# computational-cell-analytics/micro-sam

Hardware: AMD Instinct MI355X
Metric: 1024^2 tiles/s embed+AMG (vit_b bf16) (higher is better)
Workload: dtype bf16 image encoder (patch embedding + neck, 1.2 % of its flops, on hi+lo operand pairs of that type), fp16 mask decoder (16-bit MFMA operands, fp32 accumulation); 1 GPU; configs[1]: vit_b, 1024x1024 uint8 synthetic tiles, batched embedding precompute + AutomaticMaskGenerator (32x32 grid, multimask, default thresholds); encoder_batch=16, distinct_tiles_per_gpu=256, weights=seeded synthetic checkpoint (synthetic.py variant 'cells'), decode_lanes=3

## Files before the change

### micro_sam_amd/build.py

```python
import os
import subprocess
import sys

HERE = os.path.dirname(os.path.abspath(__file__))
CSRC = os.path.join(HERE, "csrc")
LIB_DIR = os.path.join(HERE, "lib")
LIB_PATH = os.path.join(LIB_DIR, "libmsam_hip.so")
SOURCES = ["gemm.hip", "norm.hip", "attention.hip", "decoder.hip", "postprocess.hip", "encoder.hip", "segment.hip", "wsgemm.hip", "declayer.hip", "decfold.hip", "decfold_tok.hip", "upfused.hip", "image.hip", "train.hip", "amgselect.hip", "watershed.hip", "strict.hip", "objfeat.hip", "matching.hip", "labelprops.hip", "propagate.hip", "embedpca.hip", "semloss.hip", "depthconv.hip"]
ARCH = "gfx950"


def _hipcc() -> str:
    for cand in (os.environ.get("HIPCC"), "/opt/rocm/bin/hipcc", "hipcc"):
        if cand and (os.path.isabs(cand) and os.path.exists(cand) or not os.path.isabs(cand)):
            return cand
    return "hipcc"


def needs_build() -> bool:
    if not os.path.exists(LIB_PATH):
        return True
    t = os.path.getmtime(LIB_PATH)
    deps = [os.path.join(CSRC, f) for f in os.listdir(CSRC)] + [os.path.join(HERE, "..", "include", "msam_hip.h")]
    return any(os.path.getmtime(d) > t for d in deps if os.path.exists(d))


def variant_path(variant: str = "") -> str:
    return LIB_PATH if not variant else os.path.join(LIB_DIR, f"libmsam_hip_{variant}.so")


def build(force: bool = False, verbose: bool = True, variant: str = "", experiments: bool = False) -> str:
    os.makedirs(LIB_DIR, exist_ok=True)
    marker = os.path.join(LIB_DIR, ".experiments")
    if experiments or os.path.exists(marker):
        force = True
        if experiments:
            open(marker, "w").close()
        else:
            os.remove(marker)
    if variant:
        return _build_variant(variant, force, verbose)
    if not force and not needs_build():
        return LIB_PATH
    objs = []
    for src in SOURCES:
        path = os.path.join(CSRC, src)
        if not os.path.exists(path):
            continue
        obj = os.path.join(LIB_DIR, src.replace(".hip", ".o"))
        if force or not os.path.exists(obj) or os.path.getmtime(obj) < max(
                os.path.getmtime(path), os.path.getmtime(os.path.join(CSRC, "common.h")),
                os.path.getmtime(os.path.join(HERE, "..", "include", "msam_hip.h"))):
            cmd = [_hipcc(), f"--offload-arch={ARCH}", "-O3", "-std=c++17", "-fPIC", "-c", path, "-o", obj]
            if experiments:
                cmd.insert(-4, "-DMSAM_EXPERIMENTS=1")
            if verbose:
                print(" ".join(cmd), flush=True)
            subprocess.check_call(cmd)
        objs.append(obj)
    cmd = [_hipcc(), f"--offload-arch={ARCH}", "-shared", "-fPIC", *objs, "-o", LIB_PATH]
    if verbose:
        print(" ".join(cmd), flush=True)
    subprocess.check_call(cmd)
    return LIB_PATH


def _build_variant(variant: str, force: bool, verbose: bool) -> str:
    if variant != "decbf16":
        raise ValueError(f"unknown build variant {variant!r}")
    out = variant_path(variant)
    deps = [os.path.join(CSRC, f) for f in os.listdir(CSRC)]
    if not force and os.path.exists(out) and all(os.path.getmtime(d) <= os.path.getmtime(out) for d in deps):
        return out
    objs = []
    for src in SOURCES:
        obj = os.path.join(LIB_DIR, src.replace(".hip", f".{variant}.o"))
        cmd = [_hipcc(), f"--offload-arch={ARCH}", "-O3", "-std=c++17", "-fPIC", "-DMSAM_DEC_F16=0", "-c", os.path.join(CSRC, src),
               "-o", obj]
        if verbose:
            print(" ".join(cmd), flush=True)
        subprocess.check_call(cmd)
        objs.append(obj)
    subprocess.check_call([_hipcc(), f"--offload-arch={ARCH}", "-shared", "-fPIC", *objs, "-o", out])
    return out


if __name__ == "__main__":
    print(build(force="--force" in sys.argv, variant="decbf16" if "--dec-bf16" in sys.argv else "", experiments="--experiments" in sys.argv))
```

### micro_sam_amd/csrc/decfold.hip

```cpp
#include "common.h"
#include "../../include/msam_hip.h"
#include <string>

void msam_set_error(const char* msg);
int msam_check_launch(const char* what);
void msam_profile_mark2(void* stream, int begin, double flops, double bytes, int family);

namespace {

constexpr int T = 4096, C = 256, CI = 128, TK = 32, NTHR = 256;
constexpr int SUBT = 1024 + 32;
constexpr int KEYS_BYTES = 16 * SUBT, TAB_BYTES = TK * CI * 2, BUF_BYTES = KEYS_BYTES + TAB_BYTES;
constexpr float NEG_BIG = -1.0e30f;
#ifndef FOLD_ATTN_DMA_DEFAULT
#define FOLD_ATTN_DMA_DEFAULT 0
#endif

typedef short s16x4_t __attribute__((ext_vector_type(4)));

MSAM_DEVINL uint2 lds_tr16(const unsigned char* p) {
    s16x4_t v = __builtin_amdgcn_ds_read_tr16_b64_v4i16((s16x4_t __attribute__((address_space(3)))*)p);
    return __builtin_bit_cast(uint2, v);
}

// ... 523 lines not shown
#undef FI_TAB
#undef I2T_STAMP
}

__global__ __launch_bounds__(256) void fold_v_kernel(const u16* __restrict__ vtok, const u16* __restrict__ wo, int Nt,
                                                     u16* __restrict__ vfoldT) {
    __shared__ float v[8][CI];
    const int p = blockIdx.x, c = threadIdx.x;
    for (int i = c; i < 8 * CI; i += 256) {
        const int t = i >> 7, d = i & (CI - 1);
        v[t][d] = t < Nt ? d2f(vtok[((long)p * Nt + t) * CI + d]) : 0.f;
    }
    __syncthreads();
    u16* dst = vfoldT + ((long)p * C + c) * 64;
    for (int h = 0; h < 8; ++h) {
        const uint4 w0 = *(const uint4*)(wo + (long)c * CI + h * 16), w1 = *(const uint4*)(wo + (long)c * CI + h * 16 + 8);
        const uint32_t ww[8] = {w0.x, w0.y, w0.z, w0.w, w1.x, w1.y, w1.z, w1.w};
        float wf[16];
#pragma unroll
        for (int x = 0; x < 8; ++x) { wf[2 * x] = d2f((u16)(ww[x] & 0xffff)); wf[2 * x + 1] = d2f((u16)(ww[x] >> 16)); }
        uint32_t pk[4];
#pragma unroll
        for (int t2 = 0; t2 < 4; ++t2) {
            float a0 = 0.f, a1 = 0.f;
#pragma unroll
            for (int d = 0; d < 16; ++d) { a0 = fmaf(wf[d], v[2 * t2][h * 16 + d], a0); a1 = fmaf(wf[d], v[2 * t2 + 1][h * 16 + d], a1); }
            pk[t2] = pack2d(a0, a1);
        }
        *(uint4*)(dst + h * 8) = make_uint4(pk[0], pk[1], pk[2], pk[3]);
    }
}

int key_splits(int P) {
    int ks = 1;
    while (P * ks < 512 && ks < 16) ks *= 2;
    return ks;
}

}

extern "C" int64_t msam_t2i_fold_workspace_bytes(int32_t P) {
    const long ks = key_splits(P);
    return (long)P * 64 * C * 2 + (long)P * ks * 64 * C * 4 + (long)P * ks * 64 * 2 * 4;
}

extern "C" int msam_t2i_fold_attention(const void* keys, int32_t kv_shared, const void* qtok, int32_t P, int32_t Nt,
                                       const void* wk, const void* tabk, const void* wv, const float* bv, void* out,
                                       void* workspace, int64_t workspace_bytes, void* stream) {
    if (!keys || !qtok || !wk || !tabk || !wv || !bv || !out || !workspace || P <= 0) {
        msam_set_error("msam_t2i_fold_attention: null argument");
        return 1;
    }
    if (Nt < 1 || Nt > 8) { msam_set_error("msam_t2i_fold_attention: 1 <= Nt <= 8 tokens per prompt"); return 1; }
    if (workspace_bytes < msam_t2i_fold_workspace_bytes(P)) { msam_set_error("msam_t2i_fold_attention: workspace too small"); return 1; }
    hipStream_t s = (hipStream_t)stream;
    const int KS = key_splits(P);
    char* wp = (char*)workspace;
    u16* qprime = (u16*)wp; wp += (long)P * 64 * C * 2;
    float* opart = (float*)wp; wp += (long)P * KS * 64 * C * 4;
    float* stats = (float*)wp;
    hipLaunchKernelGGL(fold_q_kernel, dim3(P * 8), dim3(256), 0, s, (const u16*)qtok, (const u16*)wk, Nt, qprime);
    if (int e = msam_check_launch("fold_q")) return e;
    FoldArgs a{};
    a.keys = (const u16*)keys; a.kv_shared = kv_shared & 1; a.blocked = (kv_shared >> 1) & 1; a.qprime = qprime; a.qtok = (const u16*)qtok; a.Nt = Nt;
    a.tabk = (const u16*)tabk; a.nitems = P * KS; a.KS = KS; a.opart = opart; a.stats = stats;
    a.wv = (const u16*)wv; a.bv = bv; a.out = (u16*)out;
    int dev = 0, cus = 256;
    (void)hipGetDevice(&dev);
    (void)hipDeviceGetAttribute(&cus, hipDeviceAttributeMultiprocessorCount, dev);
    const int grid = a.nitems < 2 * cus ? a.nitems : 2 * cus;
    const double flops = (double)P * T * (2.0 * 64 * C * 2 + 2.0 * 64 * 32);
    const double bytes = (double)((kv_shared & 1) ? 1 : P) * T * C * 2 + (KS > 1 ? (double)P * KS * 64 * C * 4 : 0.0);
    msam_profile_mark2(stream, 1, flops, bytes, 3);
    if (g_fold_attn_dma && !a.blocked) {
        const int grid3 = a.nitems < 3 * cus ? a.nitems : 3 * cus;
        hipLaunchKernelGGL(fold_attn_kernel<true>, dim3(grid3), dim3(NTHR), 0, s, a);
    } else {
        hipLaunchKernelGGL(fold_attn_kernel<false>, dim3(grid), dim3(NTHR), 0, s, a);
    }
    msam_profile_mark2(stream, 0, flops, bytes, 3);
    if (int e = msam_check_launch("fold_attn")) return e;
    if (KS == 1) return 0;
    hipLaunchKernelGGL(fold_finish_kernel, dim3(P * 8), dim3(128), 0, s, opart, stats, KS, Nt, (const u16*)wv, bv, (u16*)out);
    return msam_check_launch("fold_finish");
}

int64_t msam_i2t_tok_workspace_bytes(int32_t P);
int msam_i2t_tok_layer(const void* xin, int32_t x_shared, const void* ktok, const void* vtok, int32_t P, int32_t Nt,
                       const void* wq, const void* tabq, const void* wo, const float* bo, const float* ln_w,
                       const float* ln_b, float ln_eps, void* out, void* workspace, int KS, void* stream);
extern int g_tune_i2t_variant;

extern "C" int64_t msam_i2t_fold_workspace_bytes(int32_t P) {
    const int64_t a = (int64_t)P * 64 * C * 2 * 2, b = msam_i2t_tok_workspace_bytes(P);
    return a > b ? a : b;
}

extern "C" int msam_i2t_fold_layer(const void* xin, int32_t x_shared, const void* ktok, const void* vtok, int32_t P,
                                   int32_t Nt, const void* wq, const void* tabq, const void* wo, const float* bo,
                                   const float* ln_w, const float* ln_b, float ln_eps, void* out, void* workspace,
                                   int64_t workspace_bytes, void* stream) {
    if (!xin || !ktok || !vtok || !wq || !tabq || !wo || !bo || !ln_w || !ln_b || !out || !workspace || P <= 0) {
        msam_set_error("msam_i2t_fold_layer: null argument");
        return 1;
    }
    if (Nt < 1 || Nt > 8) { msam_set_error("msam_i2t_fold_layer: 1 <= Nt <= 8 tokens per prompt"); return 1; }
    if (workspace_bytes < msam_i2t_fold_workspace_bytes(P)) { msam_set_error("msam_i2t_fold_layer: workspace too small"); return 1; }
    if (g_tune_i2t_variant == 1)
        return msam_i2t_tok_layer(xin, x_shared, ktok, vtok, P, Nt, wq, tabq, wo, bo, ln_w, ln_b, ln_eps, out, workspace,
                                  key_splits(P), stream);
    hipStream_t s = (hipStream_t)stream;
    u16* kfold = (u16*)workspace;
    u16* vfoldT = kfold + (long)P * 64 * C;
    hipLaunchKernelGGL(fold_q_kernel, dim3(P * 8), dim3(256), 0, s, (const u16*)ktok, (const u16*)wq, Nt, kfold);
    if (int e = msam_check_launch("fold_k")) return e;
    hipLaunchKernelGGL(fold_v_kernel, dim3(P), dim3(256), 0, s, (const u16*)vtok, (const u16*)wo, Nt, vfoldT);
    if (int e = msam_check_launch("fold_v")) return e;
    I2tArgs a{};
    a.xin = (const u16*)xin; a.x_shared = x_shared; a.kfold = kfold; a.vfoldT = vfoldT; a.ktok = (const u16*)ktok; a.Nt = Nt;
    a.tabq = (const u16*)tabq; a.bo = bo; a.ln_w = ln_w; a.ln_b = ln_b; a.eps = ln_eps;
    a.KS = key_splits(P); a.nitems = P * a.KS; a.out = (u16*)out;
    int dev = 0, cus = 256;
    (void)hipGetDevice(&dev);
    (void)hipDeviceGetAttribute(&cus, hipDeviceAttributeMultiprocessorCount, dev);
    const int grid = a.nitems < 2 * cus ? a.nitems : 2 * cus;
    const double flops = (double)P * T * (2.0 * 64 * C * 2 + 2.0 * 64 * 32);
    const double bytes = (double)(x_shared ? 1 : P) * T * C * 2 + (double)P * T * C * 2;
    msam_profile_mark2(stream, 1, flops, bytes, 2);
    if (g_i2t_timing) hipLaunchKernelGGL(fold_i2t_kernel<true>, dim3(grid), dim3(NTHR), 0, s, a);
    else hipLaunchKernelGGL(fold_i2t_kernel<false>, dim3(grid), dim3(NTHR), 0, s, a);
    msam_profile_mark2(stream, 0, flops, bytes, 2);
    return msam_check_launch("fold_i2t");
}

extern "C" int msam_debug_i2t_timing(int32_t enable, uint64_t* host_out) {
    g_i2t_timing = enable;
    if (host_out) {
        if (hipDeviceSynchronize() != hipSuccess ||
            hipMemcpyFromSymbol(host_out, HIP_SYMBOL(g_i2t_stamps), sizeof(unsigned long long) * 64 * 12) != hipSuccess) {
            msam_set_error("msam_debug_i2t_timing: copy failed");
            return 2;
        }
    }
    return 0;
}

extern "C" int msam_fold_attn_set_dma(int32_t on) { g_fold_attn_dma = on; return 0; }

extern int g_tune_i2t_wg_per_cu, g_tune_chain_variant, g_tune_chain_tmask, g_tune_up_gelu16, g_tune_up_ln_two_pass, g_tune_up_centred;
void msam_gemm_set_dbg(int v);
void msam_gemm_set_gw(int delay, int cls);
void msam_gemm_set_g3(int delay);
void msam_gemm_set_g3_epi(int v);
extern int g_tune_tok_fuse;
extern int g_tune_mlp_split_fused;
extern int g_tune_sgemm_bufs, g_tune_srel_mfma, g_tune_sgemm_small_below, g_tune_si2t_dbg, g_tune_si2t_late_us, g_tune_sattn_allh;
int g_tune_dec_chain = 1, g_tune_dec_chain_min_p = 128;
extern "C" int msam_tune_set(const char* key, int32_t value) {
    const std::string k = key ? key : "";
    if (k == "i2t_variant") g_tune_i2t_variant = value;
    else if (k == "i2t_wg_per_cu") g_tune_i2t_wg_per_cu = value;
    else if (k == "dec_chain") g_tune_dec_chain = value;
    else if (k == "chain_variant") g_tune_chain_variant = value;
    else if (k == "chain_tmask") g_tune_chain_tmask = value;
    else if (k == "up_gelu16") g_tune_up_gelu16 = value;
    else if (k == "up_ln_two_pass") g_tune_up_ln_two_pass = value;
    else if (k == "up_centred") g_tune_up_centred = value;
    else if (k == "gemm_dbg") msam_gemm_set_dbg(value);
    else if (k == "gw_delay") msam_gemm_set_gw(value, -1);
    else if (k == "gw_class") msam_gemm_set_gw(-2, value);
    else if (k == "g3_delay") msam_gemm_set_g3(value);
    else if (k == "g3_epi") msam_gemm_set_g3_epi(value);
    else if (k == "tok_fuse") g_tune_tok_fuse = value;
    else if (k == "mlp_split_fused") g_tune_mlp_split_fused = value;
    else if (k == "dec_chain_min_p") g_tune_dec_chain_min_p = value;
    else if (k == "sgemm_bufs") g_tune_sgemm_bufs = value;
    else if (k == "srel_mfma") g_tune_srel_mfma = value;
    else if (k == "sattn_allh") g_tune_sattn_allh = value;
    else if (k == "sgemm_small_below") g_tune_sgemm_small_below = value;
    else if (k == "si2t_dbg") g_tune_si2t_dbg = value;
    else if (k == "si2t_late_us") g_tune_si2t_late_us = value;
    else { msam_set_error("msam_tune_set: unknown key"); return 1; }
    return 0;
}
```

### micro_sam_amd/csrc/gemm.hip

```cpp
#include <stdio.h>
#include <stdlib.h>
#include "common.h"
#include "../../include/msam_hip.h"

float* msam_det_workspace(size_t floats, int slot);
int msam_det_reduce(const float* parts, int nparts, long n, float* out, int accumulate, void* stream);

namespace {

constexpr int BM = 128, BN = 128, BK = 64;
constexpr int TILE_CHUNKS = BM * 8;

struct Epi {
    const float* bias; const float* table; int table_rows, table_cols; long table_ld;
    const void* resid; int resid_dtype, resid_rows; long ldr;
    int act;
    void* out; int out_dtype; long ldc;
    int out_mode; u16* q; u16* k; u16* v; int heads, head_dim, tokens;
    const float* row_scale; const float* col_scale;
    int splitk_len = 0;
    unsigned long long* trace = nullptr;
    int direct_epi = 0;
    int gw_delay = 0, gw_class = 0;
    int dbg = 0;
// ... 874 lines not shown
    } while (0)
#define LN_COMMIT(buf_)                                                                             \
    do {                                                                                            \
        uint4* la_ = ldsA + (buf_) * LM * 8; uint4* lb_ = ldsB + (buf_) * LN_ * 8;                  \
        la_[(0 * 32 + srow) * 8 + scp] = ra0; la_[(1 * 32 + srow) * 8 + scp] = ra1;                 \
        lb_[(0 * 32 + srow) * 8 + scp] = rw0; lb_[(1 * 32 + srow) * 8 + scp] = rw1;                 \
        lb_[(2 * 32 + srow) * 8 + scp] = rw2; lb_[(3 * 32 + srow) * 8 + scp] = rw3;                 \
        lb_[(4 * 32 + srow) * 8 + scp] = rw4; lb_[(5 * 32 + srow) * 8 + scp] = rw5;                 \
        lb_[(6 * 32 + srow) * 8 + scp] = rw6; lb_[(7 * 32 + srow) * 8 + scp] = rw7;                 \
    } while (0)
    LN_ISSUE(0);
    LN_COMMIT(0);
    __syncthreads();
    const int fr = lane & 15, fg = lane >> 4;
    for (int kt = 0; kt < nk; ++kt) {
        const int buf = kt & 1;
        if (kt + 1 < nk) LN_ISSUE(kt + 1);
        const uint4* la = ldsA + buf * LM * 8; const uint4* lb = ldsB + buf * LN_ * 8;
#pragma unroll
        for (int ks = 0; ks < 2; ++ks) {
            uint4 a[4], b[4];
#pragma unroll
            for (int i = 0; i < 4; ++i) {
                const int row = i * 16 + fr;
                a[i] = la[row * 8 + ((ks * 4 + fg) ^ swz(row))];
                const int col = wave * 64 + i * 16 + fr;
                b[i] = lb[col * 8 + ((ks * 4 + fg) ^ swz(col))];
            }
#pragma unroll
            for (int i = 0; i < 4; ++i)
#pragma unroll
                for (int j = 0; j < 4; ++j) acc[i][j] = F16 ? mfma16h(a[i], b[j], acc[i][j]) : mfma16(a[i], b[j], acc[i][j]);
        }
        if (kt + 1 < nk) LN_COMMIT(buf ^ 1);
        __syncthreads();
    }
#undef LN_ISSUE
#undef LN_COMMIT
    float* ldsC = (float*)dyn_lds;
#pragma unroll
    for (int i = 0; i < 4; ++i)
#pragma unroll
        for (int j = 0; j < 4; ++j)
#pragma unroll
            for (int r = 0; r < 4; ++r) ldsC[(i * 16 + fg * 4 + r) * LN_ + wave * 64 + j * 16 + fr] = acc[i][j][r];
    __syncthreads();

    const int col = lane * 4;
    float bias4[4] = {0.f, 0.f, 0.f, 0.f};
    if (e.bias) { float4 b = *(const float4*)(e.bias + col); bias4[0] = b.x; bias4[1] = b.y; bias4[2] = b.z; bias4[3] = b.w; }
    const bool use_table = e.table && col < e.table_cols;
    float lw[4] = {1.f, 1.f, 1.f, 1.f}, lb4[4] = {0.f, 0.f, 0.f, 0.f};
    if (ln.mode) {
        const int lc = ln.mode == 2 ? (col & 63) : col;
        float4 w4 = *(const float4*)(ln.ln_w + lc), b4 = *(const float4*)(ln.ln_b + lc);
        lw[0] = w4.x; lw[1] = w4.y; lw[2] = w4.z; lw[3] = w4.w; lb4[0] = b4.x; lb4[1] = b4.y; lb4[2] = b4.z; lb4[3] = b4.w;
    }
    for (int pass = 0; pass < 16; ++pass) {
        const int lr = pass * 4 + wave;
        const int row = m0 + lr;
        if (row >= M) break;
        float4 c = *(const float4*)(ldsC + lr * LN_ + col);
        float v[4] = {c.x + bias4[0], c.y + bias4[1], c.z + bias4[2], c.w + bias4[3]};
        if (use_table) {
            float4 t = *(const float4*)(e.table + (long)(row % e.table_rows) * e.table_ld + col);
            v[0] += t.x; v[1] += t.y; v[2] += t.z; v[3] += t.w;
        }
        if (e.resid_dtype) {
            const int rr = e.resid_rows ? (row % e.resid_rows) : row;
            if (e.resid_dtype == MSAM_F32) {
                float4 t = *(const float4*)((const float*)e.resid + (long)rr * e.ldr + col);
                v[0] += t.x; v[1] += t.y; v[2] += t.z; v[3] += t.w;
            } else {
                uint2 t = *(const uint2*)((const u16*)e.resid + (long)rr * e.ldr + col);
                v[0] += load16((u16)(t.x & 0xffff), e.resid_dtype); v[1] += load16((u16)(t.x >> 16), e.resid_dtype);
                v[2] += load16((u16)(t.y & 0xffff), e.resid_dtype); v[3] += load16((u16)(t.y >> 16), e.resid_dtype);
            }
        }
        if (ln.mode) {
            const float s = (v[0] + v[1]) + (v[2] + v[3]);
            const float inv_n = ln.mode == 1 ? (1.0f / 256.0f) : (1.0f / 64.0f);
            const float mean = (ln.mode == 1 ? wave_sum64(s) : wave_sum_xor16(s)) * inv_n;
            const float d0 = v[0] - mean, d1 = v[1] - mean, d2 = v[2] - mean, d3 = v[3] - mean;
            const float q = (d0 * d0 + d1 * d1) + (d2 * d2 + d3 * d3);
            const float var = (ln.mode == 1 ? wave_sum64(q) : wave_sum_xor16(q)) * inv_n;
            const float rstd = 1.0f / sqrtf(var + ln.eps);
            v[0] = d0 * rstd * lw[0] + lb4[0]; v[1] = d1 * rstd * lw[1] + lb4[1];
            v[2] = d2 * rstd * lw[2] + lb4[2]; v[3] = d3 * rstd * lw[3] + lb4[3];
            if (ln.mode == 2) { v[0] = gelu_erf(v[0]); v[1] = gelu_erf(v[1]); v[2] = gelu_erf(v[2]); v[3] = gelu_erf(v[3]); }
        }
        if (e.act == MSAM_ACT_GELU) { v[0] = gelu_erf(v[0]); v[1] = gelu_erf(v[1]); v[2] = gelu_erf(v[2]); v[3] = gelu_erf(v[3]); }
        else if (e.act == MSAM_ACT_RELU) { v[0] = fmaxf(v[0], 0.f); v[1] = fmaxf(v[1], 0.f); v[2] = fmaxf(v[2], 0.f); v[3] = fmaxf(v[3], 0.f); }
        if (e.out_dtype == MSAM_F32) {
            *(float4*)((float*)e.out + (long)row * e.ldc + col) = make_float4(v[0], v[1], v[2], v[3]);
        } else {
            uint2 pk; pk.x = pack16(v[0], v[1], e.out_dtype); pk.y = pack16(v[2], v[3], e.out_dtype);
            *(uint2*)((u16*)e.out + (long)row * e.ldc + col) = pk;
        }
        if (ln.out_b) {
            uint2 pk; pk.x = pack16(v[0], v[1], ln.dt16); pk.y = pack16(v[2], v[3], ln.dt16);
            *(uint2*)(ln.out_b + (long)row * LN_ + col) = pk;
        }
        if (ln.out_a) {
            float4 t = make_float4(0.f, 0.f, 0.f, 0.f);
            if (ln.add) t = *(const float4*)(ln.add + (long)row * LN_ + col);
            uint2 pk; pk.x = pack16(v[0] + t.x, v[1] + t.y, ln.dt16); pk.y = pack16(v[2] + t.z, v[3] + t.w, ln.dt16);
            *(uint2*)(ln.out_a + (long)row * LN_ + col) = pk;
        }
    }
}

thread_local char g_err[512] = "";

}

extern "C" const char* msam_last_error(void) { return g_err; }
extern "C" int msam_abi_version(void) { return 1; }

void msam_set_error(const char* msg) {
    int i = 0;
    for (; msg[i] && i < 510; ++i) g_err[i] = msg[i];
    g_err[i] = 0;
}

int msam_check_launch(const char* what) {
    hipError_t err = hipGetLastError();
    if (err != hipSuccess) {
        char buf[400];
        snprintf(buf, sizeof(buf), "%s: %s", what, hipGetErrorString(err));
        msam_set_error(buf);
        return 2;
    }
    return 0;
}

namespace {
struct ProfSlot { hipEvent_t a, b; double flops, bytes; int family; };
constexpr int PROF_MAX = 4096;
ProfSlot g_prof[PROF_MAX];
int g_prof_n = 0, g_prof_on = 0, g_prof_init = 0;
}

extern "C" int msam_profile_collect_family(int32_t* launches, double* ms, double* flops, double* bytes);

static int msam_num_cus() {
    static int cus = 0;
    if (cus <= 0) {
        int dev = 0;
        (void)hipGetDevice(&dev);
        if (hipDeviceGetAttribute(&cus, hipDeviceAttributeMultiprocessorCount, dev) != hipSuccess || cus <= 0) cus = 256;
    }
    return cus;
}
extern "C" int msam_gemm_set_trace(void* p) { g_gw_trace = (unsigned long long*)p; return 0; }
void msam_gemm_set_gw(int delay, int cls) { if (delay >= -1) g_tune_gw_delay = delay; if (cls >= 0) g_tune_gw_class = cls; }
void msam_gemm_set_g3(int delay) { g_tune_g3_delay = delay; }
void msam_gemm_set_g3_epi(int v) { g_tune_g3_epi = v; }
void msam_gemm_set_dbg(int v) { g_tune_gemm_dbg = v; }
extern "C" int msam_gemm256_set_staging(int staging) {
    if (staging < -1 || staging > 4) { msam_set_error("msam_gemm256_set_staging: -1 (default), 0, 1, 2, 3 or 4"); return 1; }
    g_gemm256_staging = staging;
    return 0;
}

extern "C" int msam_profile_enable(int on) {
    if (on && !g_prof_init) {
        for (int i = 0; i < PROF_MAX; ++i) {
            if (hipEventCreate(&g_prof[i].a) != hipSuccess || hipEventCreate(&g_prof[i].b) != hipSuccess) {
                msam_set_error("msam_profile_enable: hipEventCreate failed");
                return 2;
            }
        }
        g_prof_init = 1;
    }
    g_prof_on = on; g_prof_n = 0;
    return 0;
}

extern "C" int msam_profile_collect(int32_t* launches, double* total_ms, double* total_flops) {
    int32_t n[MSAM_PROFILE_FAMILIES]; double ms[MSAM_PROFILE_FAMILIES], fl[MSAM_PROFILE_FAMILIES], by[MSAM_PROFILE_FAMILIES];
    if (int e = msam_profile_collect_family(n, ms, fl, by)) return e;
    int32_t nn = 0; double tm = 0, tf = 0;
    for (int f = 0; f < MSAM_PROFILE_FAMILIES; ++f) { nn += n[f]; tm += ms[f]; tf += fl[f]; }
    if (launches) *launches = nn;
    if (total_ms) *total_ms = tm;
    if (total_flops) *total_flops = tf;
    return 0;
}

extern "C" int msam_profile_collect_family(int32_t* launches, double* ms, double* flops, double* bytes) {
    for (int f = 0; f < MSAM_PROFILE_FAMILIES; ++f) { launches[f] = 0; ms[f] = 0; flops[f] = 0; bytes[f] = 0; }
    for (int i = 0; i < g_prof_n; ++i) {
        if (hipEventSynchronize(g_prof[i].b) != hipSuccess) { msam_set_error("msam_profile_collect: sync failed"); return 2; }
        float t = 0.f;
        hipEventElapsedTime(&t, g_prof[i].a, g_prof[i].b);
        const int f = (unsigned)g_prof[i].family < MSAM_PROFILE_FAMILIES ? g_prof[i].family : 1;
        ++launches[f]; ms[f] += t; flops[f] += g_prof[i].flops; bytes[f] += g_prof[i].bytes;
    }
    g_prof_n = 0;
    return 0;
}

void msam_profile_mark2(void* stream, int begin, double flops, double bytes, int family) {
    if (!g_prof_on || g_prof_n >= PROF_MAX) return;
    if (begin) {
        g_prof[g_prof_n].flops = flops; g_prof[g_prof_n].bytes = bytes; g_prof[g_prof_n].family = family;
        (void)hipEventRecord(g_prof[g_prof_n].a, (hipStream_t)stream);
    } else { (void)hipEventRecord(g_prof[g_prof_n].b, (hipStream_t)stream); ++g_prof_n; }
}
void msam_profile_mark(void* stream, int begin, double flops) { msam_profile_mark2(stream, begin, flops, 0.0, 1); }

extern "C" int msam_gemm_bf16(const msam_gemm_t* p, void* stream) {
    if (!p || !p->A || !p->W) { msam_set_error("msam_gemm_bf16: null operand"); return 1; }
    if (p->M <= 0 || p->N <= 0 || p->K <= 0 || p->N % BN != 0 || p->K % BK != 0) {
        msam_set_error("msam_gemm_bf16: need M > 0, N % 128 == 0, K % 64 == 0");
        return 1;
    }
    if ((p->lda % 8) || (p->ldw % 8)) { msam_set_error("msam_gemm_bf16: lda/ldw must be multiples of 8"); return 1; }
    if (p->out_mode == 0 && (p->ldc % 4)) { msam_set_error("msam_gemm_bf16: ldc must be a multiple of 4"); return 1; }
    if (p->out_mode == 3 && (!p->out || p->ldc != 3L * p->N || p->N % 4 || p->out_dtype == MSAM_F32 || p->ln_mode || p->split_k > 1 || p->a_dtype == MSAM_FP8)) {
        msam_set_error("msam_gemm_bf16: out_mode 3 (hi + lo pairs) needs a 16-bit output with ldc == 3 N, no fused LayerNorm / split-K / fp8");
        return 1;
    }
    if (p->out_mode < 0 || p->out_mode > 3) { msam_set_error("msam_gemm_bf16: out_mode is 0 .. 3"); return 1; }
    if ((p->table && ((p->table_cols % 4) || (p->table_ld % 4))) || (p->resid && (p->ldr % 4))) {
        msam_set_error("msam_gemm_bf16: table_cols/table_ld/ldr must be multiples of 4");
        return 1;
    }
    if (p->out_mode == 0 && !p->out) { msam_set_error("msam_gemm_bf16: null output"); return 1; }
    if (p->out_mode == 1 && (!p->q || !p->k || !p->v || p->heads * p->head_dim * 3 != p->N || p->head_dim % 4)) {
        msam_set_error("msam_gemm_bf16: bad qkv-split arguments");
        return 1;
    }
    if (p->out_mode == 2 && (!p->k || !p->v || p->N != 256 || p->tokens % 128 || p->M % p->tokens)) {
        msam_set_error("msam_gemm_bf16: bad kv-split arguments (N == 256, tokens % 128 == 0, M % tokens == 0)");
        return 1;
    }
    Epi e;
    e.bias = p->bias; e.table = p->table; e.table_rows = p->table_rows > 0 ? p->table_rows : 1;
    e.table_cols = p->table_cols; e.table_ld = p->table_ld;
    e.resid = p->resid; e.resid_dtype = p->resid ? p->resid_dtype : 0; e.resid_rows = p->resid_rows; e.ldr = p->ldr;
    e.act = p->act; e.out = p->out; e.out_dtype = p->out_dtype; e.ldc = p->ldc;
    e.out_mode = p->out_mode; e.q = (u16*)p->q; e.k = (u16*)p->k; e.v = (u16*)p->v;
    e.heads = p->heads; e.head_dim = p->head_dim; e.tokens = p->tokens;
    e.row_scale = nullptr; e.col_scale = nullptr;
    e.splitk_len = 0;
    e.dbg = MSAM_EXPERIMENTS ? g_tune_gemm_dbg : 0;
    hipStream_t s = (hipStream_t)stream;
    if (p->ln_mode && p->a_dtype == MSAM_FP8) { msam_set_error("msam_gemm_bf16(fp8): no fused LayerNorm epilogue"); return 1; }
    const bool f16 = p->a_dtype == MSAM_F16;
    if (p->ln_mode) {
        if (p->N != 256 || p->out_mode != 0 || !p->ln_w || !p->ln_b || p->ln_mode < 0 || p->ln_mode > 2) {
            msam_set_error("msam_gemm_bf16: fused LayerNorm needs N == 256, plain output and ln_w / ln_b");
            return 1;
        }
        static bool attr_set = false;
        constexpr int LN_LDS = 2 * (64 * 8 + 256 * 8) * 16;
        if (!attr_set) {
            if (hipFuncSetAttribute((const void*)gemm_ln_kernel<false>, hipFuncAttributeMaxDynamicSharedMemorySize, LN_LDS) != hipSuccess ||
                hipFuncSetAttribute((const void*)gemm_ln_kernel<true>, hipFuncAttributeMaxDynamicSharedMemorySize, LN_LDS) != hipSuccess) {
                msam_set_error("msam_gemm_bf16: cannot raise the dynamic LDS limit");
                return 2;
            }
            attr_set = true;
        }
        if ((p->ln_out_a || p->ln_out_b) && p->ln_mode != 1) { msam_set_error("msam_gemm_bf16: ln_out_a / ln_out_b go with ln_mode 1"); return 1; }
        EpiLN ln{p->ln_w, p->ln_b, p->ln_eps, p->ln_mode, p->ln_add, (u16*)p->ln_out_a, (u16*)p->ln_out_b, f16 ? MSAM_F16 : MSAM_BF16};
        const bool prof_ln = g_prof_on && g_prof_n < PROF_MAX;
        if (prof_ln) {
            g_prof[g_prof_n].flops = 2.0 * p->M * (double)p->N * p->K; g_prof[g_prof_n].bytes = 0; g_prof[g_prof_n].family = 5;
            (void)hipEventRecord(g_prof[g_prof_n].a, s);
        }
        if (f16) hipLaunchKernelGGL(gemm_ln_kernel<true>, dim3((p->M + 63) / 64), dim3(256), LN_LDS, s, (const u16*)p->A, (long)p->lda,
                                    (const u16*)p->W, (long)p->ldw, p->M, p->K, e, ln);
        else hipLaunchKernelGGL(gemm_ln_kernel<false>, dim3((p->M + 63) / 64), dim3(256), LN_LDS, s, (const u16*)p->A, (long)p->lda,
                                (const u16*)p->W, (long)p->ldw, p->M, p->K, e, ln);
        if (prof_ln) { (void)hipEventRecord(g_prof[g_prof_n].b, s); ++g_prof_n; }
        return msam_check_launch("msam_gemm_bf16(ln)");
    }
    const bool prof = g_prof_on && g_prof_n < PROF_MAX;
    if (p->a_dtype == MSAM_FP8) {
        if (p->N % G2 || p->K % 128 || (p->lda % 16) || (p->ldw % 16) || p->ln_mode || p->out_mode == 2 || p->table ||
            p->use_glds || !p->row_scale || !p->col_scale ||
            (p->resid && (p->resid_dtype != MSAM_F32 || p->resid_rows))) {
            msam_set_error("msam_gemm_bf16(fp8): need N % 256 == 0, K % 128 == 0, lda / ldw % 16 == 0, row_scale and col_scale, plain or qkv-split "
                           "output, fp32 residual without row wrap, no table");
            return 1;
        }
        static bool attr8 = false;
        if (!attr8) {
            if (hipFuncSetAttribute((const void*)gemm256_kernel<1, true>, hipFuncAttributeMaxDynamicSharedMemorySize, G2_LDS) != hipSuccess) {
                msam_set_error("msam_gemm_bf16: cannot raise the dynamic LDS limit");
                return 2;
            }
            attr8 = true;
        }
        e.row_scale = p->row_scale; e.col_scale = p->col_scale;
        if (prof) {
            g_prof[g_prof_n].flops = 2.0 * p->M * (double)p->N * p->K; g_prof[g_prof_n].bytes = 0; g_prof[g_prof_n].family = 0;
            (void)hipEventRecord(g_prof[g_prof_n].a, s);
        }
        const int tiles8 = ((p->M + G2 - 1) / G2) * (p->N / G2);
        hipLaunchKernelGGL((gemm256_kernel<1, true>), dim3(tiles8), dim3(512), G2_LDS, s, (const u16*)p->A, (long)p->lda,
                           (const u16*)p->W, (long)p->ldw, p->M, p->N, p->K, e);
        if (prof) { (void)hipEventRecord(g_prof[g_prof_n].b, s); ++g_prof_n; }
        return msam_check_launch("msam_gemm_bf16(fp8)");
    }
    int tiles = ((p->M + BM - 1) / BM) * (p->N / BN);
    static int use256 = -1, staging256 = 0;
    if (use256 < 0) {
        const char* v = getenv("MSAM_GEMM256"); use256 = v ? atoi(v) : 1;
        const char* st = getenv("MSAM_GEMM256_STAGING"); staging256 = st ? atoi(st) : G2_DEFAULT_STAGING;
    }
    if (g_gemm256_staging >= 0) staging256 = g_gemm256_staging;
    if (!MSAM_EXPERIMENTS && (staging256 < 0 || staging256 > 3)) staging256 = G2_DEFAULT_STAGING;
    if (MSAM_EXPERIMENTS && use256 && staging256 == 4 && (double)p->M * p->lda * 2 < 2147483648.0 && (double)p->N * p->ldw * 2 < 2147483648.0 && p->split_k <= 1 && (!f16 || p->out_dtype != MSAM_BF16) && !p->use_glds &&
        ((p->M + G2 - 1) / G2) * (p->N / G2) >= 256 && p->N % GW_BN == 0 && p->K % GW_BK == 0 && p->lda % 8 == 0 && p->ldw % 8 == 0 &&
        p->out_mode != 2 && p->out_mode != 3 && !p->table && (!p->resid || (p->resid_dtype == MSAM_F32 && !p->resid_rows))) {
        static bool attr2w = false;
        if (!attr2w) {
            if (hipFuncSetAttribute((const void*)gemm2w_kernel<false>, hipFuncAttributeMaxDynamicSharedMemorySize, GW_LDS) != hipSuccess ||
                hipFuncSetAttribute((const void*)gemm2w_kernel<true>, hipFuncAttributeMaxDynamicSharedMemorySize, GW_LDS) != hipSuccess) {
                msam_set_error("msam_gemm_bf16: cannot raise the dynamic LDS limit");
                return 2;
            }
            attr2w = true;
            if (getenv("MSAM_GEMM_OCC")) {
                int nb = -1;
                (void)hipOccupancyMaxActiveBlocksPerMultiprocessor(&nb, (const void*)gemm2w_kernel<false>, 256, GW_LDS);
                fprintf(stderr, "gemm2w_kernel: %d workgroups per CU (dynamic LDS %d)\n", nb, GW_LDS);
            }
        }
        if (prof) {
            g_prof[g_prof_n].flops = 2.0 * p->M * (double)p->N * p->K; g_prof[g_prof_n].bytes = 0; g_prof[g_prof_n].family = 0;
            (void)hipEventRecord(g_prof[g_prof_n].a, s);
        }
        const int tiles2w = ((p->M + GW_BM - 1) / GW_BM) * (p->N / GW_BN);
        const int gmul = (g_tune_gemm_dbg >> 8) & 15 ? (g_tune_gemm_dbg >> 8) & 15 : 2;
        const int grid2w = tiles2w < gmul * msam_num_cus() ? tiles2w : gmul * msam_num_cus();
        e.gw_class = g_tune_gw_class;
        e.trace = g_gw_trace;
        e.gw_delay = g_tune_gw_delay >= 0 ? g_tune_gw_delay : (p->K / GW_BK) / 4;
        if (f16)
            hipLaunchKernelGGL(gemm2w_kernel<true>, dim3(grid2w), dim3(256), GW_LDS, s, (const u16*)p->A, (long)p->lda, (const u16*)p->W,
                               (long)p->ldw, p->M, p->N, p->K, e);
        else
            hipLaunchKernelGGL(gemm2w_kernel<false>, dim3(grid2w), dim3(256), GW_LDS, s, (const u16*)p->A, (long)p->lda, (const u16*)p->W,
                               (long)p->ldw, p->M, p->N, p->K, e);
        if (prof) { (void)hipEventRecord(g_prof[g_prof_n].b, s); ++g_prof_n; }
        return msam_check_launch("msam_gemm_bf16(2w)");
    }
    if (use256 && p->split_k <= 1 && (!f16 || p->out_dtype != MSAM_BF16) && !p->use_glds && ((p->M + G2 - 1) / G2) * (p->N / G2) >= 256 && p->N % G2 == 0 &&
        p->out_mode != 2 && p->out_mode != 3 && !p->table && (!p->resid || (p->resid_dtype == MSAM_F32 && !p->resid_rows))) {
        static bool attr256 = false;
        if (!attr256) {
            if (hipFuncSetAttribute((const void*)gemm256_kernel<0>, hipFuncAttributeMaxDynamicSharedMemorySize, G2_LDS) != hipSuccess ||
                hipFuncSetAttribute((const void*)gemm256_kernel<1>, hipFuncAttributeMaxDynamicSharedMemorySize, G2_LDS) != hipSuccess ||
                hipFuncSetAttribute((const void*)gemm256_kernel<2>, hipFuncAttributeMaxDynamicSharedMemorySize, G2_LDS) != hipSuccess ||
                hipFuncSetAttribute((const void*)gemm256_kernel<3>, hipFuncAttributeMaxDynamicSharedMemorySize, G2_LDS) != hipSuccess ||
                hipFuncSetAttribute((const void*)gemm256_kernel<3, false, true>, hipFuncAttributeMaxDynamicSharedMemorySize, G2_LDS) != hipSuccess) {
                msam_set_error("msam_gemm_bf16: cannot raise the dynamic LDS limit");
                return 2;
            }
            attr256 = true;
        }
        if (prof) {
            g_prof[g_prof_n].flops = 2.0 * p->M * (double)p->N * p->K; g_prof[g_prof_n].bytes = 0; g_prof[g_prof_n].family = 0;
            (void)hipEventRecord(g_prof[g_prof_n].a, s);
        }
        const int tiles256 = ((p->M + G2 - 1) / G2) * (p->N / G2);
        e.gw_class = msam_num_cus();
        e.gw_delay = g_tune_g3_delay >= 0 ? g_tune_g3_delay : 0;
        e.direct_epi = (MSAM_EXPERIMENTS && (p->out_dtype == MSAM_F32 || (p->out_dtype == MSAM_F16) == f16)) ? g_tune_g3_epi : 0;
#define G2_GO(ST_) hipLaunchKernelGGL(gemm256_kernel<ST_>, dim3(tiles256), dim3(512), G2_LDS, s, (const u16*)p->A, (long)p->lda, \
                                     (const u16*)p->W, (long)p->ldw, p->M, p->N, p->K, e)
        if (f16)
            hipLaunchKernelGGL((gemm256_kernel<3, false, true>), dim3(tiles256), dim3(512), G2_LDS, s, (const u16*)p->A, (long)p->lda,
                               (const u16*)p->W, (long)p->ldw, p->M, p->N, p->K, e);
        else if (staging256 == 1) G2_GO(1); else if (staging256 == 2) G2_GO(2); else if (staging256 == 3) G2_GO(3); else G2_GO(0);
#undef G2_GO
        if (prof) { (void)hipEventRecord(g_prof[g_prof_n].b, s); ++g_prof_n; }
        return msam_check_launch("msam_gemm_bf16(256)");
    }
    if (p->split_k > 1) {
        if (p->out_mode != 0 || p->out_dtype != MSAM_F32 || p->bias || p->table || p->resid || p->act || p->ldc != p->N ||
            p->K % (p->split_k * BK)) {
            msam_set_error("msam_gemm_bf16(split_k): plain fp32 output with ldc == N, no bias / table / residual / activation, K % (split_k * 64) == 0");
            return 1;
        }
        float* parts = msam_det_workspace((size_t)p->split_k * p->M * p->N, 2);
        if (!parts) { msam_set_error("msam_gemm_bf16(split_k): cannot allocate the partial-tile workspace"); return 2; }
        e.out = parts;
        e.splitk_len = p->K / p->split_k;
        if (f16) hipLaunchKernelGGL((gemm_kernel<false, true>), dim3(tiles, p->split_k), dim3(256), 0, s, (const u16*)p->A, (long)p->lda,
                                    (const u16*)p->W, (long)p->ldw, p->M, p->N, p->K, e);
        else hipLaunchKernelGGL(gemm_kernel<false>, dim3(tiles, p->split_k), dim3(256), 0, s, (const u16*)p->A, (long)p->lda,
                                (const u16*)p->W, (long)p->ldw, p->M, p->N, p->K, e);
        if (msam_det_reduce(parts, p->split_k, (long)p->M * p->N, (float*)p->out, 0, stream)) {
            msam_set_error("msam_gemm_bf16(split_k): cannot allocate the reduction workspace");
            return 2;
        }
        return msam_check_launch("msam_gemm_bf16(split_k)");
    }
    if (prof) {
        g_prof[g_prof_n].flops = 2.0 * p->M * (double)p->N * p->K; g_prof[g_prof_n].bytes = 0; g_prof[g_prof_n].family = 5;
        (void)hipEventRecord(g_prof[g_prof_n].a, s);
    }
    if (f16)
        hipLaunchKernelGGL((gemm_kernel<false, true>), dim3(tiles), dim3(256), 0, s, (const u16*)p->A, (long)p->lda,
                           (const u16*)p->W, (long)p->ldw, p->M, p->N, p->K, e);
    else if (p->use_glds)
        hipLaunchKernelGGL(gemm_kernel<true>, dim3(tiles), dim3(256), 0, s, (const u16*)p->A, (long)p->lda,
                           (const u16*)p->W, (long)p->ldw, p->M, p->N, p->K, e);
    else
        hipLaunchKernelGGL(gemm_kernel<false>, dim3(tiles), dim3(256), 0, s, (const u16*)p->A, (long)p->lda,
                           (const u16*)p->W, (long)p->ldw, p->M, p->N, p->K, e);
    if (prof) { (void)hipEventRecord(g_prof[g_prof_n].b, s); ++g_prof_n; }
    return msam_check_launch("msam_gemm_bf16");
}

extern "C" int msam_gemm_group_bf16(const msam_gemm_t* items, int32_t n, void* stream) {
    if (!items || n <= 0 || n > MSAM_GEMM_GROUP_MAX) { msam_set_error("msam_gemm_group_bf16: 1 .. MSAM_GEMM_GROUP_MAX products"); return 1; }
    GroupArgs g{};
    int max_tiles = 0;
    double flops = 0.0;
    for (int i = 0; i < n; ++i) {
        const msam_gemm_t* p = items + i;
        if (!p->A || !p->W || p->M <= 0 || p->N <= 0 || p->K <= 0 || p->N % BN || p->K % BK || (p->lda % 8) || (p->ldw % 8) ||
            p->ln_mode || p->a_dtype == MSAM_FP8 || p->use_glds || (p->a_dtype == MSAM_F16) != (items[0].a_dtype == MSAM_F16)) {
            msam_set_error("msam_gemm_group_bf16: every product needs N % 128 == 0, K % 64 == 0, lda / ldw % 8 == 0, bf16 operands "
                           "(or fp16 for all of them), no fused LayerNorm");
            return 1;
        }
        if ((p->out_mode == 0 && (!p->out || (p->ldc % 4))) || p->out_mode == 1 ||
            (p->out_mode == 2 && (!p->k || !p->v || p->N != 256 || p->tokens % 128 || p->M % p->tokens)) || p->out_mode > 3 || p->out_mode < 0 ||
            (p->out_mode == 3 && (!p->out || p->ldc != 3L * p->N || p->N % 4 || p->out_dtype == MSAM_F32)) ||
            (p->table && ((p->table_cols % 4) || (p->table_ld % 4))) || (p->resid && (p->ldr % 4))) {
            msam_set_error("msam_gemm_group_bf16: bad output / table / residual arguments (qkv-split output is not grouped; out_mode 3 needs a "
                           "16-bit output with ldc == 3 N)");
            return 1;
        }
        GroupItem& it = g.it[i];
        it.A = (const u16*)p->A; it.lda = p->lda; it.W = (const u16*)p->W; it.ldw = p->ldw; it.M = p->M; it.N = p->N; it.K = p->K;
        Epi& e = it.e;
        e.bias = p->bias; e.table = p->table; e.table_rows = p->table_rows > 0 ? p->table_rows : 1;
        e.table_cols = p->table_cols; e.table_ld = p->table_ld;
        e.resid = p->resid; e.resid_dtype = p->resid ? p->resid_dtype : 0; e.resid_rows = p->resid_rows; e.ldr = p->ldr;
        e.act = p->act; e.out = p->out; e.out_dtype = p->out_dtype; e.ldc = p->ldc;
        e.out_mode = p->out_mode; e.q = (u16*)p->q; e.k = (u16*)p->k; e.v = (u16*)p->v;
        e.heads = p->heads; e.head_dim = p->head_dim; e.tokens = p->tokens;
        e.row_scale = nullptr; e.col_scale = nullptr;
        e.splitk_len = 0; e.dbg = 0;
        const int tiles = ((p->M + BM - 1) / BM) * (p->N / BN);
        if (tiles > max_tiles) max_tiles = tiles;
        flops += 2.0 * p->M * (double)p->N * p->K;
    }
    for (int i = n; i < MSAM_GEMM_GROUP_MAX; ++i) g.it[i] = g.it[0];
    hipStream_t s = (hipStream_t)stream;
    const bool prof = g_prof_on && g_prof_n < PROF_MAX;
    if (prof) {
        g_prof[g_prof_n].flops = flops; g_prof[g_prof_n].bytes = 0; g_prof[g_prof_n].family = 5;
        (void)hipEventRecord(g_prof[g_prof_n].a, s);
    }
    if (items[0].a_dtype == MSAM_F16) hipLaunchKernelGGL(gemm_group_kernel<true>, dim3(max_tiles, n), dim3(256), 0, s, g);
    else hipLaunchKernelGGL(gemm_group_kernel<false>, dim3(max_tiles, n), dim3(256), 0, s, g);
    if (prof) { (void)hipEventRecord(g_prof[g_prof_n].b, s); ++g_prof_n; }
    return msam_check_launch("msam_gemm_group_bf16");
}
```

Baseline: 177.6 tiles/s.

## Route small GEMMs to a new 64x64-tile kernel when tiles underfill CUs

Adds a separate GEMM kernel with 64x64 output tiles and a double-buffered register-staged K loop. Both the single and grouped bf16/fp16 GEMM entry points use it when the large-tile grid would have fewer tiles than there are CUs and the arguments fit its limits (no LayerNorm, table or split-k; ReLU or no activation; fp32 residual). The aim is to spread small decoder- and token-sized products over more workgroups so fewer CUs sit idle. The cost is less operand reuse per tile and a second code path whose epilogue has to reproduce the original one's numerics.

```diff
diff --git a/micro_sam_amd/build.py b/micro_sam_amd/build.py
--- a/micro_sam_amd/build.py
+++ b/micro_sam_amd/build.py
@@ -6,7 +6,7 @@
 CSRC = os.path.join(HERE, "csrc")
 LIB_DIR = os.path.join(HERE, "lib")
 LIB_PATH = os.path.join(LIB_DIR, "libmsam_hip.so")
-SOURCES = ["gemm.hip", "norm.hip", "attention.hip", "decoder.hip", "postprocess.hip", "encoder.hip", "segment.hip", "wsgemm.hip", "declayer.hip", "decfold.hip", "decfold_tok.hip", "upfused.hip", "image.hip", "train.hip", "amgselect.hip", "watershed.hip", "strict.hip", "objfeat.hip", "matching.hip", "labelprops.hip", "propagate.hip", "embedpca.hip", "semloss.hip", "depthconv.hip"]
+SOURCES = ["gemm.hip", "gemm_tok.hip", "norm.hip", "attention.hip", "decoder.hip", "postprocess.hip", "encoder.hip", "segment.hip", "wsgemm.hip", "declayer.hip", "decfold.hip", "decfold_tok.hip", "upfused.hip", "image.hip", "train.hip", "amgselect.hip", "watershed.hip", "strict.hip", "objfeat.hip", "matching.hip", "labelprops.hip", "propagate.hip", "embedpca.hip", "semloss.hip", "depthconv.hip"]
 ARCH = "gfx950"
 
 
diff --git a/micro_sam_amd/csrc/decfold.hip b/micro_sam_amd/csrc/decfold.hip
--- a/micro_sam_amd/csrc/decfold.hip
+++ b/micro_sam_amd/csrc/decfold.hip
@@ -699,6 +699,7 @@
 void msam_gemm_set_gw(int delay, int cls);
 void msam_gemm_set_g3(int delay);
 void msam_gemm_set_g3_epi(int v);
+void msam_gemm_set_small_tile(int v);
 extern int g_tune_tok_fuse;
 extern int g_tune_mlp_split_fused;
 extern int g_tune_sgemm_bufs, g_tune_srel_mfma, g_tune_sgemm_small_below, g_tune_si2t_dbg, g_tune_si2t_late_us, g_tune_sattn_allh;
@@ -719,6 +720,7 @@
     else if (k == "g3_delay") msam_gemm_set_g3(value);
     else if (k == "g3_epi") msam_gemm_set_g3_epi(value);
     else if (k == "tok_fuse") g_tune_tok_fuse = value;
+    else if (k == "gemm_small_tile") msam_gemm_set_small_tile(value);
     else if (k == "mlp_split_fused") g_tune_mlp_split_fused = value;
     else if (k == "dec_chain_min_p") g_tune_dec_chain_min_p = value;
     else if (k == "sgemm_bufs") g_tune_sgemm_bufs = value;
diff --git a/micro_sam_amd/csrc/gemm.hip b/micro_sam_amd/csrc/gemm.hip
--- a/micro_sam_amd/csrc/gemm.hip
+++ b/micro_sam_amd/csrc/gemm.hip
@@ -1050,6 +1050,10 @@
     }
     return cus;
 }
+bool msam_gemm_tok_ok(const msam_gemm_t* p);
+int msam_gemm_tok(const msam_gemm_t* items, int n, int variant, void* stream);
+int g_tune_gemm_small_tile = 1;
+void msam_gemm_set_small_tile(int v) { g_tune_gemm_small_tile = v; }
 extern "C" int msam_gemm_set_trace(void* p) { g_gw_trace = (unsigned long long*)p; return 0; }
 void msam_gemm_set_gw(int delay, int cls) { if (delay >= -1) g_tune_gw_delay = delay; if (cls >= 0) g_tune_gw_class = cls; }
 void msam_gemm_set_g3(int delay) { g_tune_g3_delay = delay; }
@@ -1205,6 +1209,7 @@
         return msam_check_launch("msam_gemm_bf16(fp8)");
     }
     int tiles = ((p->M + BM - 1) / BM) * (p->N / BN);
+    if (g_tune_gemm_small_tile > 0 && tiles < msam_num_cus() && msam_gemm_tok_ok(p)) return msam_gemm_tok(p, 1, g_tune_gemm_small_tile, stream);
     static int use256 = -1, staging256 = 0;
     if (use256 < 0) {
         const char* v = getenv("MSAM_GEMM256"); use256 = v ? atoi(v) : 1;
@@ -1320,7 +1325,8 @@
 extern "C" int msam_gemm_group_bf16(const msam_gemm_t* items, int32_t n, void* stream) {
     if (!items || n <= 0 || n > MSAM_GEMM_GROUP_MAX) { msam_set_error("msam_gemm_group_bf16: 1 .. MSAM_GEMM_GROUP_MAX products"); return 1; }
     GroupArgs g{};
-    int max_tiles = 0;
+    int max_tiles = 0, sum_tiles = 0;
+    bool small_ok = g_tune_gemm_small_tile > 0;
     double flops = 0.0;
     for (int i = 0; i < n; ++i) {
         const msam_gemm_t* p = items + i;
@@ -1351,8 +1357,11 @@
         e.splitk_len = 0; e.dbg = 0;
         const int tiles = ((p->M + BM - 1) / BM) * (p->N / BN);
         if (tiles > max_tiles) max_tiles = tiles;
+        sum_tiles += tiles;
+        small_ok = small_ok && msam_gemm_tok_ok(p);
         flops += 2.0 * p->M * (double)p->N * p->K;
     }
+    if (small_ok && sum_tiles < msam_num_cus()) return msam_gemm_tok(items, n, g_tune_gemm_small_tile, stream);
     for (int i = n; i < MSAM_GEMM_GROUP_MAX; ++i) g.it[i] = g.it[0];
     hipStream_t s = (hipStream_t)stream;
     const bool prof = g_prof_on && g_prof_n < PROF_MAX;
diff --git a/micro_sam_amd/csrc/gemm_tok.hip b/micro_sam_amd/csrc/gemm_tok.hip
--- /dev/null
+++ b/micro_sam_amd/csrc/gemm_tok.hip
@@ -0,0 +1,243 @@
+#include "common.h"
+#include "../../include/msam_hip.h"
+
+void msam_set_error(const char* msg);
+int msam_check_launch(const char* what);
+void msam_profile_mark2(void* stream, int begin, double flops, double bytes, int family);
+
+namespace {
+
+constexpr int TK = 64;
+
+struct TokItem {
+    const u16* A; const u16* W; const float* bias; const float* resid; void* out;
+    long lda, ldw, ldr, ldc;
+    int M, N, K, act, out_dtype, out_mode;
+};
+struct TokArgs { TokItem it[MSAM_GEMM_GROUP_MAX]; };
+
+MSAM_DEVINL uint32_t tok_pack16(float lo, float hi, int dt) { return dt == MSAM_F16 ? pack2h(lo, hi) : pack2bf(lo, hi); }
+MSAM_DEVINL float tok_load16(u16 v, int dt) { return dt == MSAM_F16 ? h2f(v) : bf2f(v); }
+
+template <int TBM, int TBN, bool F16>
+MSAM_DEVINL void gemm_tok_body(const TokItem& t, int bid_in) {
+    constexpr int WN = 128 / TBM, TN = TBN / WN, FN = TN / 16;
+    constexpr int PA = TBM / 32, PW = TBN / 32;
+    constexpr int A_CH = TBM * 8, W_CH = TBN * 8;
+    static_assert(2 * (A_CH + W_CH) * 16 >= TBM * TBN * 4, "the fp32 C tile is staged through the operand buffers");
+    __shared__ __attribute__((aligned(16))) uint4 lds[2][A_CH + W_CH];
+
+    const u16* __restrict__ A = t.A; const u16* __restrict__ W = t.W;
+    const int M = t.M, N = t.N, K = t.K;
+    const int tid = threadIdx.x, lane = tid & 63, wave = tid >> 6;
+    const int tiles_n = N / TBN, tiles_m = (M + TBM - 1) / TBM;
+    int nwg = tiles_m * tiles_n, bid = bid_in;
+    {
+        int xcd = bid & 7, q = nwg >> 3, r = nwg & 7;
+        bid = (xcd < r ? xcd * (q + 1) : r * (q + 1) + (xcd - r) * q) + (bid >> 3);
+    }
+    const int tile_m = bid / tiles_n, tile_n = bid % tiles_n;
+    const int m0 = tile_m * TBM, n0 = tile_n * TBN;
+    const int wm = wave / WN, wn = wave % WN;
+
+    const int srow = tid >> 3, scp = tid & 7;
+    int aoff[PA], woff[PW];
+#pragma unroll
+    for (int p = 0; p < PA; ++p) {
+        const int row = p * 32 + srow, gc = scp ^ swz(row);
+        aoff[p] = (int)((long)min(m0 + row, M - 1) * t.lda * 2 + gc * 16);
+    }
+#pragma unroll
+    for (int p = 0; p < PW; ++p) {
+        const int row = p * 32 + srow, gc = scp ^ swz(row);
+        woff[p] = (int)((long)(n0 + row) * t.ldw * 2 + gc * 16);
+    }
+    const rsrc_t ra = make_rsrc(A, (uint32_t)(((long)(M - 1) * t.lda + K) * 2));
+    const rsrc_t rw = make_rsrc(W, (uint32_t)(((long)(N - 1) * t.ldw + K) * 2));
+
+    f32x4_t acc[2][FN];
+#pragma unroll
+    for (int i = 0; i < 2; ++i)
+#pragma unroll
+        for (int j = 0; j < FN; ++j) acc[i][j] = (f32x4_t){0.f, 0.f, 0.f, 0.f};
+
+    const int fr = lane & 15, fg = lane >> 4;
+    auto compute = [&](int buf) {
+        const uint4* la = &lds[buf][0];
+        const uint4* lw = &lds[buf][A_CH];
+#pragma unroll
+        for (int ks = 0; ks < 2; ++ks) {
+            uint4 a[2], b[FN];
+#pragma unroll
+            for (int i = 0; i < 2; ++i) {
+                const int row = wm * 32 + i * 16 + fr;
+                a[i] = la[row * 8 + ((ks * 4 + fg) ^ swz(row))];
+            }
+#pragma unroll
+            for (int j = 0; j < FN; ++j) {
+                const int col = wn * TN + j * 16 + fr;
+                b[j] = lw[col * 8 + ((ks * 4 + fg) ^ swz(col))];
+            }
+#pragma unroll
+            for (int i = 0; i < 2; ++i)
+#pragma unroll
+                for (int j = 0; j < FN; ++j) acc[i][j] = F16 ? mfma16h(a[i], b[j], acc[i][j]) : mfma16(a[i], b[j], acc[i][j]);
+        }
+    };
+
+    const int nk = K / TK;
+    uint4 xa[PA], xw[PW], ya[PA], yw[PW];
+    auto load = [&](uint4 (&a)[PA], uint4 (&w)[PW], int kt) {
+        const int so = kt * TK * 2;
+#pragma unroll
+        for (int p = 0; p < PA; ++p) a[p] = buf_load16(ra, aoff[p], so);
+#pragma unroll
+        for (int p = 0; p < PW; ++p) w[p] = buf_load16(rw, woff[p], so);
+    };
+    auto commit = [&](const uint4 (&a)[PA], const uint4 (&w)[PW], int buf) {
+#pragma unroll
+        for (int p = 0; p < PA; ++p) lds[buf][(p * 32 + srow) * 8 + scp] = a[p];
+#pragma unroll
+        for (int p = 0; p < PW; ++p) lds[buf][A_CH + (p * 32 + srow) * 8 + scp] = w[p];
+    };
+    load(xa, xw, 0);
+    commit(xa, xw, 0);
+    load(xa, xw, min(1, nk - 1));
+    __syncthreads();
+    int kt = 0;
+    while (true) {
+        load(ya, yw, min(kt + 2, nk - 1));
+        compute(kt & 1);
+        if (kt + 1 < nk) commit(xa, xw, (kt & 1) ^ 1);
+        __syncthreads();
+        if (++kt >= nk) break;
+        load(xa, xw, min(kt + 2, nk - 1));
+        compute(kt & 1);
+        if (kt + 1 < nk) commit(ya, yw, (kt & 1) ^ 1);
+        __syncthreads();
+        if (++kt >= nk) break;
+    }
+    wait_vmem_all();
+
+    float* ldsC = (float*)&lds[0][0];
+#pragma unroll
+    for (int i = 0; i < 2; ++i)
+#pragma unroll
+        for (int j = 0; j < FN; ++j)
+#pragma unroll
+            for (int r = 0; r < 4; ++r)
+                ldsC[(wm * 32 + i * 16 + fg * 4 + r) * TBN + wn * TN + j * 16 + fr] = acc[i][j][r];
+    __syncthreads();
+
+    constexpr int TPR = TBN / 4, RPP = 256 / TPR, NPASS = TBM / RPP;
+    const int c4 = (tid % TPR) * 4;
+    const int col = n0 + c4;
+    float bias4[4] = {0.f, 0.f, 0.f, 0.f};
+    if (t.bias) { float4 b = *(const float4*)(t.bias + col); bias4[0] = b.x; bias4[1] = b.y; bias4[2] = b.z; bias4[3] = b.w; }
+    const int lr0 = tid / TPR;
+    float4 rt[NPASS];
+#pragma unroll
+    for (int pass = 0; pass < NPASS; ++pass) {
+        const int row = min(m0 + pass * RPP + lr0, M - 1);
+        float4 s = make_float4(0.f, 0.f, 0.f, 0.f);
+        if (t.resid) {
+            const float4 u = *(const float4*)(t.resid + (long)row * t.ldr + col);
+            s.x += u.x; s.y += u.y; s.z += u.z; s.w += u.w;
+        }
+        rt[pass] = s;
+    }
+    const int odt = t.out_dtype;
+#pragma unroll
+    for (int pass = 0; pass < NPASS; ++pass) {
+        const int lr = pass * RPP + lr0;
+        const int row = m0 + lr;
+        if (row >= M) break;
+        float4 c = *(const float4*)(ldsC + lr * TBN + c4);
+        float v[4] = {(c.x + bias4[0]) + rt[pass].x, (c.y + bias4[1]) + rt[pass].y, (c.z + bias4[2]) + rt[pass].z,
+                      (c.w + bias4[3]) + rt[pass].w};
+        if (t.act == MSAM_ACT_RELU) {
+#pragma unroll
+            for (int x = 0; x < 4; ++x) v[x] = fmaxf(v[x], 0.f);
+        }
+        if (t.out_mode == 0) {
+            if (odt == MSAM_F32) {
+                *(float4*)((float*)t.out + (long)row * t.ldc + col) = make_float4(v[0], v[1], v[2], v[3]);
+            } else {
+                uint2 pk; pk.x = tok_pack16(v[0], v[1], odt); pk.y = tok_pack16(v[2], v[3], odt);
+                *(uint2*)((u16*)t.out + (long)row * t.ldc + col) = pk;
+            }
+        } else {
+            uint2 hi, lo;
+            hi.x = tok_pack16(v[0], v[1], odt); hi.y = tok_pack16(v[2], v[3], odt);
+            lo.x = tok_pack16(v[0] - tok_load16((u16)(hi.x & 0xffff), odt), v[1] - tok_load16((u16)(hi.x >> 16), odt), odt);
+            lo.y = tok_pack16(v[2] - tok_load16((u16)(hi.y & 0xffff), odt), v[3] - tok_load16((u16)(hi.y >> 16), odt), odt);
+            u16* o = (u16*)t.out + (long)row * t.ldc + col;
+            const long third = t.ldc / 3;
+            *(uint2*)o = hi; *(uint2*)(o + third) = lo; *(uint2*)(o + 2 * third) = hi;
+        }
+    }
+}
+
+template <int TBM, int TBN, bool F16>
+__global__ __launch_bounds__(256) void gemm_tok_kernel(TokArgs g) {
+#if defined(__HIP_DEVICE_COMPILE__)
+    (void)g;
+    typedef const __attribute__((address_space(4))) TokItem* ItemPtr;
+    const TokItem t = *((ItemPtr)__builtin_amdgcn_kernarg_segment_ptr() + blockIdx.y);
+#else
+    const TokItem t = g.it[blockIdx.y];
+#endif
+    const int tiles = ((t.M + TBM - 1) / TBM) * (t.N / TBN);
+    if ((int)blockIdx.x >= tiles) return;
+    gemm_tok_body<TBM, TBN, F16>(t, (int)blockIdx.x);
+}
+
+}
+
+bool msam_gemm_tok_ok(const msam_gemm_t* p) {
+    if (p->ln_mode || p->split_k > 1 || p->use_glds || p->table || (p->a_dtype != MSAM_F16 && p->a_dtype != MSAM_BF16 && p->a_dtype != 0))
+        return false;
+    if (p->act != 0 && p->act != MSAM_ACT_RELU) return false;
+    if (p->resid && (p->resid_dtype != MSAM_F32 || p->resid_rows)) return false;
+    if (p->out_mode != 0 && p->out_mode != 3) return false;
+    if (!p->out || p->N % 64 || p->K % TK) return false;
+    if (((double)(p->M - 1) * p->lda + p->K) * 2 >= 2147483648.0 || ((double)(p->N - 1) * p->ldw + p->K) * 2 >= 2147483648.0) return false;
+    return true;
+}
+
+#ifndef MSAM_EXPERIMENTS
+#define MSAM_EXPERIMENTS 0
+#endif
+int msam_gemm_tok(const msam_gemm_t* items, int n, int variant, void* stream) {
+    TokArgs g{};
+    if (!MSAM_EXPERIMENTS) variant = 1;
+    const int tbm = variant == 3 ? 32 : 64, tbn = variant == 2 || variant == 3 ? 128 : 64;
+    int max_tiles = 0;
+    double flops = 0.0;
+    for (int i = 0; i < n; ++i) {
+        const msam_gemm_t* p = items + i;
+        TokItem& t = g.it[i];
+        t.A = (const u16*)p->A; t.W = (const u16*)p->W; t.bias = p->bias; t.resid = (const float*)p->resid; t.out = p->out;
+        t.lda = p->lda; t.ldw = p->ldw; t.ldr = p->ldr; t.ldc = p->ldc;
+        t.M = p->M; t.N = p->N; t.K = p->K; t.act = p->act; t.out_dtype = p->out_dtype; t.out_mode = p->out_mode;
+        const int tiles = ((p->M + tbm - 1) / tbm) * (p->N / tbn);
+        if (tiles > max_tiles) max_tiles = tiles;
+        flops += 2.0 * p->M * (double)p->N * p->K;
+    }
+    for (int i = n; i < MSAM_GEMM_GROUP_MAX; ++i) g.it[i] = g.it[0];
+    hipStream_t s = (hipStream_t)stream;
+    const bool f16 = items[0].a_dtype == MSAM_F16;
+    msam_profile_mark2(stream, 1, flops, 0.0, 5);
+#define TOK_GO(BM_, BN_)                                                                                            \
+    do {                                                                                                            \
+        if (f16) hipLaunchKernelGGL((gemm_tok_kernel<BM_, BN_, true>), dim3(max_tiles, n), dim3(256), 0, s, g);     \
+        else hipLaunchKernelGGL((gemm_tok_kernel<BM_, BN_, false>), dim3(max_tiles, n), dim3(256), 0, s, g);        \
+    } while (0)
+#if MSAM_EXPERIMENTS
+    if (variant == 2) TOK_GO(64, 128); else if (variant == 3) TOK_GO(32, 128); else
+#endif
+    TOK_GO(64, 64);
+#undef TOK_GO
+    msam_profile_mark2(stream, 0, flops, 0.0, 5);
+    return msam_check_launch("msam_gemm_tok");
+}
```

After: 178.0 tiles/s (median of 4 runs). About the same (+0.2%).
